# OpenDriveLab/ST-P3

Measured on AMD Instinct MI355X. Metric: BEV samples/sec (6-cam x 3-frame fwd+bwd), higher is better.
Workload: dtype bf16 convs / f32 voxel pool; 1 GPU; BASELINE configs[2]: batch=4/GPU, 6-cam 224x480, T=3, full STP3 fwd+bwd with segmentation + pedestrian + hdmap + depth CE + instance centerness/offset + flow losses, grad-clip 5, Adam; EfficientNet-B4, D=48, C=64, BEV 200x200; global_batch=4, parallelism=dp1, launch=hipgraph

## Files before the change

include/stp3_hip.h:

```cpp
#ifndef STP3_HIP_H
#define STP3_HIP_H

#include <stddef.h>
#include <stdint.h>

#ifdef __cplusplus
extern "C" {
#endif

#define STP3_OK          0
#define STP3_EINVAL   (-10001)
#define STP3_EUNSUP   (-10002)
#define STP3_ENOSPACE (-10003)

#define STP3_DTYPE_F32  0
#define STP3_DTYPE_BF16 1

typedef struct stp3_lift_dims {
    int32_t B, T, N;
    int32_t D, fH, fW;
    int32_t C;
    int32_t X, Y, Z;
} stp3_lift_dims;

// ... 99 lines not shown
    int32_t act, res_mode;
    int32_t has_sbias, has_oscale;
    int32_t cpad;
} stp3_bn_dims;

int stp3_bn_workspace_bytes(const stp3_bn_dims* dims, size_t* bytes);
int stp3_bn_stats(const stp3_bn_dims* dims, const void* x, const float* sbias, void* workspace,
                  size_t workspace_bytes, float* sums, void* stream);
int stp3_bn_apply_fwd(const stp3_bn_dims* dims, const void* x, const float* sbias, const void* res,
                      const float* oscale, const float* sums, double count, const float* gamma,
                      const float* beta, float eps, float momentum, float* running_mean,
                      float* running_var, float* save_mean, float* save_invstd, void* y, void* stream);
int stp3_bn_bwd_reduce(const stp3_bn_dims* dims, const void* dy, const void* x, const float* sbias,
                       const void* res, const float* oscale, const float* mean, const float* invstd,
                       const float* gamma, const float* beta, void* workspace, size_t workspace_bytes,
                       float* sample_sums, float* sums, void* stream);
int stp3_bn_apply_bwd(const stp3_bn_dims* dims, const void* dy, const void* x, const float* sbias,
                      const void* res, const float* oscale, const float* mean, const float* invstd,
                      const float* gamma, const float* beta, const float* sums, double count, void* dx,
                      void* dres, void* stream);
int stp3_bn_fwd_train(const stp3_bn_dims* dims, const void* x, const float* sbias, const void* res,
                      const float* oscale, const float* gamma, const float* beta, float eps, float momentum,
                      float* running_mean, float* running_var, float* stat_buf, void* workspace,
                      size_t workspace_bytes, void* y, void* stream);
int stp3_bn_bwd_train(const stp3_bn_dims* dims, const void* dy, const void* x, const float* sbias,
                      const void* res, const float* oscale, const float* mean, const float* invstd,
                      const float* gamma, const float* beta, void* workspace, size_t workspace_bytes,
                      float* sum_buf, void* dx, void* dres, void* stream);

int stp3_bn_dsbias(int32_t N, int32_t C, int32_t rows, const float* sample_sums, const float* gsums, double count,
                   const float* gamma, const float* invstd, float* dsbias, void* stream);
int stp3_sum_n(int32_t n, int64_t numel, int32_t dtype, const void* const* src, void* y, void* stream);
int stp3_sum_n_plane(int32_t n, int64_t numel, int32_t dtype, const void* const* src, const void* plane, int64_t per_sample,
                     int32_t C, void* y, void* stream);

int stp3_linear_fwd(int32_t M, int32_t K, int32_t N, const float* x, const float* w, int32_t ldw, const float* b, float* y,
                    void* stream);
int stp3_linear_bwd(int32_t M, int32_t K, int32_t N, const float* dy, const float* x, const float* w, int32_t ldw, float* dx,
                    float* dw, int32_t lddw, float* db, void* stream);

typedef struct stp3_conv_dims {
    int32_t N, H, W, Cin;
    int32_t Ho, Wo, Cout;
    int32_t KH, KW, stride;
    int32_t pad_h, pad_w, dil_h, dil_w;
    int32_t ldx, ldy;
    int32_t out_dtype, has_bias;
} stp3_conv_dims;

int stp3_conv2d_fwd_workspace(const stp3_conv_dims* dims, size_t* bytes);
int stp3_conv2d_fwd(const stp3_conv_dims* dims, const void* x, const void* w, const float* bias, void* y,
                    float* sums, void* workspace, size_t workspace_bytes, void* stream);

int stp3_conv2d_fwd_stats(const stp3_conv_dims* dims, const void* x, const void* w, float* sums, void* workspace,
                          size_t workspace_bytes, void* stream);
int stp3_conv2d_fwd_bnact(const stp3_conv_dims* dims, const void* x, const void* w, const float* coef, int32_t act, void* y,
                          void* stream);
int stp3_conv2d_bn_bwd_reduce(const stp3_conv_dims* dims, const void* x, const void* w, const void* dz, int32_t ldz,
                              const float* coef, int32_t act, float* sums, void* workspace, size_t workspace_bytes,
                              void* stream);
int stp3_conv2d_bn_bwd_apply(const stp3_conv_dims* dims, const void* x, const void* w, const void* dz, int32_t ldz,
                             const float* coef, int32_t act, const float* gsums, double count, void* dy, void* stream);
int stp3_conv2d_bn_bwd_apply_dx(const stp3_conv_dims* dims, const void* x, const void* w, const void* dz, int32_t ldz,
                                const float* coef, int32_t act, const float* gsums, double count, void* dy, void* dx,
                                int32_t lddx, const void* add, int32_t ldadd, void* stream);

int stp3_conv2d_fwd_add(const stp3_conv_dims* dims, const void* x, const void* w, const float* bias, const void* add,
                        int32_t ldadd, void* y, void* stream);

int stp3_conv2d_wgrad_workspace(const stp3_conv_dims* dims, size_t* bytes);
int stp3_conv2d_wgrad(const stp3_conv_dims* dims, const void* dy, const void* x, float* dw, void* workspace,
                      size_t workspace_bytes, void* stream);

#define STP3_WGRAD_BATCH_MAX 96
typedef struct stp3_wgrad_job {
    const void* partials;
    float* dw;
    int64_t numel;
    int32_t splits;
    int32_t reserved;
} stp3_wgrad_job;
int stp3_conv2d_wgrad_partials(const stp3_conv_dims* dims, const void* dy, const void* x, void* partials,
                               size_t partials_bytes, int32_t* splits, void* stream);
int stp3_conv2d_wgrad_reduce_batch(int32_t n, const stp3_wgrad_job* jobs, void* stream);

typedef struct stp3_se_dims {
    int32_t N, rows, C, ld;
    int32_t dtype;
} stp3_se_dims;

int stp3_se_workspace_bytes(const stp3_se_dims* dims, size_t* bytes);
int stp3_se_pool(const stp3_se_dims* dims, const void* x, const void* dy, void* workspace, size_t workspace_bytes,
                 float* out, void* stream);
int stp3_se_scale(const stp3_se_dims* dims, const void* x, const float* gate, const float* add, void* y, void* stream);

typedef struct stp3_se_mlp_dims {
    int32_t N, C, S;
    float inv_rows;
} stp3_se_mlp_dims;

int stp3_se_mlp_fwd(const stp3_se_mlp_dims* dims, const float* pooled_sum, const float* w1, const float* b1,
                    const float* w2, const float* b2, float* z1, float* gate, void* stream);
int stp3_se_mlp_bwd(const stp3_se_mlp_dims* dims, const float* dgate, const float* gate, const float* pooled_sum,
                    const float* z1, const float* w1, const float* w2, float* dz2, float* dz1, float* dpooled,
                    float* dw1, float* db1, float* dw2, float* db2, void* stream);

// ... 230 lines not shown
```

st-p3_amd/csrc/stp3_conv.hip:

```cpp
#include <hip/hip_runtime.h>
#include <stdint.h>
#include <stdlib.h>
#include <string.h>

#include "stp3_cdna.h"
#include "stp3_hip.h"

namespace {

typedef __attribute__((ext_vector_type(8))) __bf16 bf16x8;
typedef __attribute__((ext_vector_type(4))) float f32x4;
typedef __attribute__((ext_vector_type(16))) float f32x16;

struct ConvDims {
    int N, H, W, Cin, Ho, Wo, Cout;
    int KH, KW, stride, pad_h, pad_w, dil_h, dil_w;
    int ldx, ldy;
    int out_f32, has_bias;
    int M;
    int kchunks;
    int Ktot;
};

union Frag {
// ... 348 lines not shown
                *reinterpret_cast<uint4*>(yo + (size_t)m * d.ldy + co) =
                    make_uint4(pack_bf16(out[0], out[1]), pack_bf16(out[2], out[3]), pack_bf16(out[4], out[5]),
                               pack_bf16(out[6], out[7]));
            }
        }
    }
    if (MODE == kModeBwdReduce) {
        uint16_t* gt = tile + kBM * ldt;
        for (int e = tid; e < kBM * (BN / 8); e += 256) {
            const int p = e / (BN / 8), c = (e - p * (BN / 8)) * 8;
            const int m = m0 + p, co = co0 + c;
            uint4 g = make_uint4(0u, 0u, 0u, 0u);
            if (m < d.M && co < d.Cout) g = *reinterpret_cast<const uint4*>(ep.dz + (size_t)m * ep.ldz + co);
            *reinterpret_cast<uint4*>(gt + p * ldt + c) = g;
        }
        __syncthreads();
        float* red = reinterpret_cast<float*>(smem + 2 * kBM * ldt * 2);
        const int c = tid % BN, part = tid / BN;
        constexpr int kParts = 256 / BN, kRows = kBM / kParts;
        float s1 = 0.f, s2 = 0.f;
        if (co0 + c < d.Cout) {
            const float cs = ep.coef[co0 + c], ct = ep.coef[d.Cout + co0 + c];
            const float mu = ep.coef[2 * d.Cout + co0 + c], is = ep.coef[3 * d.Cout + co0 + c];
            for (int p = part * kRows; p < (part + 1) * kRows; ++p) {
                if (m0 + p < d.M) {
                    const float e0 = bf2f(tile[p * ldt + c]);
                    const float gg = bf2f(gt[p * ldt + c]) * epi_act_grad<ACT>(fmaf(e0, cs, ct));
                    s1 += gg;
                    s2 = fmaf(gg, (e0 - mu) * is, s2);
                }
            }
        }
        red[(part * 2) * BN + c] = s1;
        red[(part * 2 + 1) * BN + c] = s2;
        __syncthreads();
        if (tid < 2 * BN) {
            const int k = tid / BN, cc = tid - k * BN;
            float t = 0.f;
#pragma unroll
            for (int q = 0; q < kParts; ++q) t += red[(q * 2 + k) * BN + cc];
            if (co0 + cc < d.Cout) stat_partial[((size_t)tile_m * 2 + k) * d.Cout + co0 + cc] = t;
        }
    }
    if ((MODE == kModePlain || MODE == kModeStats) && stat_partial) {
        float* red = reinterpret_cast<float*>(smem + kBM * ldt * 2);
        const int c = tid % BN, part = tid / BN;
        constexpr int kParts = 256 / BN, kRows = kBM / kParts;
        float s1 = 0.f, s2 = 0.f;
        for (int p = part * kRows; p < (part + 1) * kRows; ++p) {
            if (m0 + p < d.M) {
                const float v = bf2f(tile[p * ldt + c]);
                s1 += v;
                s2 += v * v;
            }
        }
        red[(part * 2) * BN + c] = s1;
        red[(part * 2 + 1) * BN + c] = s2;
        __syncthreads();
        if (tid < 2 * BN) {
            const int k = tid / BN, cc = tid - k * BN;
            float t = 0.f;
#pragma unroll
            for (int q = 0; q < kParts; ++q) t += red[(q * 2 + k) * BN + cc];
            if (co0 + cc < d.Cout) stat_partial[((size_t)tile_m * 2 + k) * d.Cout + co0 + cc] = t;
        }
    }
}

struct Chan8 {
    stp3_f32x2 cs[4], ct[4], mu[4], is[4], a2[4], a3[4];
    uint32_t keep[4];
};

template <int MODE>
__device__ __forceinline__ void load_chan8(Chan8& k, const EpiArgs& ep, int Cout, int c, bool ok) {
#pragma unroll
    for (int r = 0; r < 4; ++r)
#pragma unroll
        for (int h = 0; h < 2; ++h) {
            k.cs[r][h] = k.ct[r][h] = k.mu[r][h] = k.is[r][h] = k.a2[r][h] = k.a3[r][h] = 0.f;
            if (MODE == kModeAffine && h == 0)
                k.keep[r] = (c + 2 * r < ep.cvalid ? 0x0000ffffu : 0u) | (c + 2 * r + 1 < ep.cvalid ? 0xffff0000u : 0u);
            if (MODE >= kModeBnAct && ok) {
                const int cc = c + 2 * r + h;
                k.cs[r][h] = ep.coef[cc];
                k.ct[r][h] = ep.coef[Cout + cc];
                if (MODE == kModeAffine) continue;
                k.mu[r][h] = ep.coef[2 * Cout + cc];
                k.is[r][h] = ep.coef[3 * Cout + cc];
                if (MODE == kModeBwdApply) {
                    const float k0 = ep.gsums[cc] * ep.inv_count, k1 = ep.gsums[Cout + cc] * ep.inv_count;
                    k.a2[r][h] = -(k.cs[r][h] * k.is[r][h]) * k1;
                    k.a3[r][h] = -k.cs[r][h] * k0 - k.a2[r][h] * k.mu[r][h];
                }
            }
        }
}

template <int MODE>
__device__ __forceinline__ void epi8(const uint32_t (&wds)[4], const uint32_t (&gds)[4], const Chan8& k, int act,
                                     stp3_f32x2 (&s1)[4], stp3_f32x2 (&s2)[4], uint32_t (&ow)[4], int res_mode = STP3_RES_NONE) {
#pragma unroll
    for (int r = 0; r < 4; ++r) {
        const uint32_t wd = MODE == kModeAffine ? wds[r] & k.keep[r] : wds[r];
        const stp3_f32x2 e0 = {__uint_as_float(wd << 16), __uint_as_float(wd & 0xffff0000u)};
        if (MODE == kModePlain || MODE == kModeStats) {
// ... 619 lines not shown
    }
    float4 t;
    t.x = (s0.x + s1.x) + (s2.x + s3.x); t.y = (s0.y + s1.y) + (s2.y + s3.y);
    t.z = (s0.z + s1.z) + (s2.z + s3.z); t.w = (s0.w + s1.w) + (s2.w + s3.w);
    red[threadIdx.x] = t;
    __syncthreads();
    if (kl == 0 && i < n) {
        const float4 a = red[cg], bb = red[64 + cg], c = red[128 + cg], d = red[192 + cg];
        float4 o;
        o.x = (a.x + bb.x) + (c.x + d.x); o.y = (a.y + bb.y) + (c.y + d.y);
        o.z = (a.z + bb.z) + (c.z + d.z); o.w = (a.w + bb.w) + (c.w + d.w);
        if (i + 3 < n && ((uintptr_t)(dw + i) & 15) == 0) {
            *reinterpret_cast<float4*>(dw + i) = o;
        } else {
            const float* oe = &o.x;
            for (int e = 0; e < 4 && i + e < n; ++e) dw[i + e] = oe[e];
        }
    }
}

inline int status() {
    hipError_t e = hipGetLastError();
    return e == hipSuccess ? STP3_OK : -(int)e;
}

inline size_t igemm_lds(int bn, int steps, bool out_f32) {
    const size_t stage = (size_t)(steps > 1 ? 2 : 1) * (kBM + bn) * kBK * 2;
    const size_t tile = out_f32 ? (size_t)kBM * (bn + 8) * 4 : (size_t)kBM * (bn + 8) * 2 + 512 * sizeof(float);
    return stage > tile ? stage : tile;
}

template <int TCO, int TCI>
int wgrad_launch(const ConvDims& d, int tco, int tci, int taps, int splits, int ksteps, int fold, const void* dy,
                 const void* x, void* workspace, hipStream_t s) {
    const size_t lds = (size_t)2 * (TCO + TCI) * kBK * 2;
    const int xcd = taps <= 9 && (int64_t)tco * tci * taps * splits < (1LL << 31);
    const bool buf = (size_t)d.M * d.ldy * 2 < (1ull << 31) && (size_t)d.N * d.H * d.W * d.ldx * 2 < (1ull << 31);
    if (buf) {
        hipError_t e = hipFuncSetAttribute(reinterpret_cast<const void*>(&conv2d_wgrad_kernel<TCO, TCI, true>),
                                           hipFuncAttributeMaxDynamicSharedMemorySize, (int)lds);
        if (e != hipSuccess) return -(int)e;
        hipLaunchKernelGGL((conv2d_wgrad_kernel<TCO, TCI, true>), dim3(tco * tci, taps, splits), dim3(256), lds, s, d, tci,
                           ksteps, fold, xcd, (const uint16_t*)dy, (const uint16_t*)x, (float*)workspace);
        return STP3_OK;
    }
    hipError_t e = hipFuncSetAttribute(reinterpret_cast<const void*>(&conv2d_wgrad_kernel<TCO, TCI>),
                                       hipFuncAttributeMaxDynamicSharedMemorySize, (int)lds);
    if (e != hipSuccess) return -(int)e;
    hipLaunchKernelGGL((conv2d_wgrad_kernel<TCO, TCI>), dim3(tco * tci, taps, splits), dim3(256), lds, s, d, tci, ksteps,
                       fold, xcd, (const uint16_t*)dy, (const uint16_t*)x, (float*)workspace);
    return STP3_OK;
}

}

extern "C" {

int stp3_conv2d_fwd_workspace(const stp3_conv_dims* p, size_t* bytes) {
    if (!p || !bytes || p->N <= 0 || p->Ho <= 0 || p->Wo <= 0 || p->Cout <= 0) return STP3_EINVAL;
    const int64_t M = (int64_t)p->N * p->Ho * p->Wo;
    const size_t parts = (size_t)((M + kBM - 1) / kBM);
    if (parts > 65536) return STP3_EUNSUP;
    *bytes = (parts + (parts + 255) / 256) * 2 * p->Cout * sizeof(float);
    return STP3_OK;
}

}

namespace {

template <int BN, int MODE, int ACT>
int igemm_launch_one(const ConvDims& d, dim3 grid, size_t lds, int tiles_co, const void* x, const void* w, const float* bias,
                     void* y, float* partial, const EpiArgs& ep, hipStream_t s) {
    const bool buf = (size_t)d.N * d.H * d.W * d.ldx * 2 < (1ull << 31) && (size_t)d.Cout * d.Ktot * 2 < (1ull << 31);
    if (buf) {
        hipError_t e = hipFuncSetAttribute(reinterpret_cast<const void*>(&conv2d_igemm_kernel<BN, MODE, ACT, true>),
                                           hipFuncAttributeMaxDynamicSharedMemorySize, (int)lds);
        if (e != hipSuccess) return -(int)e;
        hipLaunchKernelGGL((conv2d_igemm_kernel<BN, MODE, ACT, true>), grid, dim3(256), lds, s, d, tiles_co, (const uint16_t*)x,
                           (const uint16_t*)w, bias, y, partial, ep);
        return STP3_OK;
    }
    hipError_t e = hipFuncSetAttribute(reinterpret_cast<const void*>(&conv2d_igemm_kernel<BN, MODE, ACT>),
                                       hipFuncAttributeMaxDynamicSharedMemorySize, (int)lds);
    if (e != hipSuccess) return -(int)e;
    hipLaunchKernelGGL((conv2d_igemm_kernel<BN, MODE, ACT>), grid, dim3(256), lds, s, d, tiles_co, (const uint16_t*)x,
                       (const uint16_t*)w, bias, y, partial, ep);
    return STP3_OK;
}

template <int BN, int MODE>
int igemm_launch_act(int act, const ConvDims& d, dim3 grid, size_t lds, int tiles_co, const void* x, const void* w,
                     const float* bias, void* y, float* partial, const EpiArgs& ep, hipStream_t s) {
    if (MODE == kModePlain || MODE == kModeStats || act == STP3_ACT_NONE)
        return igemm_launch_one<BN, MODE, STP3_ACT_NONE>(d, grid, lds, tiles_co, x, w, bias, y, partial, ep, s);
    if (act == STP3_ACT_RELU) return igemm_launch_one<BN, MODE, STP3_ACT_RELU>(d, grid, lds, tiles_co, x, w, bias, y, partial, ep, s);
    return igemm_launch_one<BN, MODE, STP3_ACT_SWISH>(d, grid, lds, tiles_co, x, w, bias, y, partial, ep, s);
}

template <int PP, int KMAX, int MODE>
int pointwise_rows_launch_one(const ConvDims& d, int ksteps, int tiles_co, unsigned nwg, size_t lds, const void* x, const void* w,
                              void* y, float* partial, const EpiArgs& ep, hipStream_t s) {
    hipError_t e = hipFuncSetAttribute(reinterpret_cast<const void*>(&pointwise_rows_kernel<PP, KMAX, MODE>),
                                       hipFuncAttributeMaxDynamicSharedMemorySize, (int)lds);
    if (e != hipSuccess) return -(int)e;
    hipLaunchKernelGGL((pointwise_rows_kernel<PP, KMAX, MODE>), dim3(nwg), dim3(256), lds, s, d, ksteps, tiles_co,
                       (const uint16_t*)x, (const uint16_t*)w, (uint16_t*)y, partial, ep);
    return STP3_OK;
}

template <int PP, int KMAX>
int pointwise_rows_launch_mode(int mode, const ConvDims& d, int ksteps, int tiles_co, unsigned nwg, size_t lds, const void* x,
                               const void* w, void* y, float* partial, const EpiArgs& ep, hipStream_t s) {
    switch (mode) {
        case kModePlain: return pointwise_rows_launch_one<PP, KMAX, kModePlain>(d, ksteps, tiles_co, nwg, lds, x, w, y, partial, ep, s);
        case kModeStats: return pointwise_rows_launch_one<PP, KMAX, kModeStats>(d, ksteps, tiles_co, nwg, lds, x, w, y, partial, ep, s);
        case kModeBnAct: return pointwise_rows_launch_one<PP, KMAX, kModeBnAct>(d, ksteps, tiles_co, nwg, lds, x, w, y, partial, ep, s);
        case kModeAffine: return pointwise_rows_launch_one<PP, KMAX, kModeAffine>(d, ksteps, tiles_co, nwg, lds, x, w, y, partial, ep, s);
        case kModeBwdReduce:
            return pointwise_rows_launch_one<PP, KMAX, kModeBwdReduce>(d, ksteps, tiles_co, nwg, lds, x, w, y, partial, ep, s);
        default: return pointwise_rows_launch_one<PP, KMAX, kModeBwdApply>(d, ksteps, tiles_co, nwg, lds, x, w, y, partial, ep, s);
    }
}

template <int KMAX, int MODE>
int pointwise_direct_launch_one(const ConvDims& d, int ksteps, unsigned gx, int* parts, const void* x, const void* w, void* y,
                                float* partial, const EpiArgs& ep, hipStream_t s) {
    static const int resident = [] {
        int per_cu = 0;
        if (hipOccupancyMaxActiveBlocksPerMultiprocessor(&per_cu, pointwise_direct_kernel<KMAX, MODE>, 256, 0) != hipSuccess || per_cu < 1)
            per_cu = 1;
        return per_cu * 256;
    }();
    const int cblocks = (d.Cout + 31) / 32;
    const int ntiles = (d.M + 31) / 32;
    int ngroups = resident * 4 / cblocks;
    if (ngroups > (int)gx) ngroups = (int)gx;
    if (ngroups > ntiles) ngroups = ntiles;
    if (ngroups < 1) ngroups = 1;
    *parts = ngroups;
// ... 9 lines not shown
    switch (mode) {
        case kModePlain: return pointwise_direct_launch_one<KMAX, kModePlain>(d, ksteps, gx, parts, x, w, y, partial, ep, s);
        case kModeStats: return pointwise_direct_launch_one<KMAX, kModeStats>(d, ksteps, gx, parts, x, w, y, partial, ep, s);
        case kModeBnAct: return pointwise_direct_launch_one<KMAX, kModeBnAct>(d, ksteps, gx, parts, x, w, y, partial, ep, s);
        case kModeAffine: return pointwise_direct_launch_one<KMAX, kModeAffine>(d, ksteps, gx, parts, x, w, y, partial, ep, s);
        case kModeBwdReduce: return pointwise_direct_launch_one<KMAX, kModeBwdReduce>(d, ksteps, gx, parts, x, w, y, partial, ep, s);
        default: return pointwise_direct_launch_one<KMAX, kModeBwdApply>(d, ksteps, gx, parts, x, w, y, partial, ep, s);
    }
}

constexpr int kPointwiseMaxCin = 128;

bool pointwise_applies(const stp3_conv_dims* p, const void* y) {
    return p->KH == 1 && p->KW == 1 && p->stride == 1 && p->pad_h == 0 && p->pad_w == 0 && p->H == p->Ho && p->W == p->Wo &&
           p->Cin <= kPointwiseMaxCin && p->Cout >= 64 && !p->has_bias && p->out_dtype == STP3_DTYPE_BF16 &&
           p->Cout % 8 == 0 && p->ldy % 8 == 0 && !((uintptr_t)y & 15);
}

int pointwise_run(const ConvDims& d, const void* x, const void* w, void* y, float* sums, float* partial, unsigned gx,
                  hipStream_t s, int mode, const EpiArgs& ep) {
    const int ksteps = (d.Cin + 15) / 16;
    int rc, parts;
    const bool rows_small = (d.Cout == 144 || d.Cout == 192) && ksteps <= 2;
    const bool rows_lines = d.Cout % 64 == 0;
    if ((rows_small || rows_lines) && d.ldy % 8 == 0 && (!mode_bwd(mode) || ep.ldz % 8 == 0)) {
        const int pp = rows_small ? d.Cout / 8 : (d.Cout % 128 == 0 ? 16 : 8), nt = (pp + 3) / 4;
        const int tiles_co = d.Cout / (pp * 8);
        if (ep.dx && !(rows_small && mode == kModeBwdApply && d.Cin <= 32)) return STP3_EUNSUP;
        const size_t lds = (size_t)nt * 32 * (ksteps * 16 + 8) * 2 + (size_t)4 * 32 * (nt * 32 + 8) * 2 +
                           (ep.dx ? (size_t)32 * (nt * 32 + 8) * 2 : 0);
        unsigned per_cu = (unsigned)((160 * 1024) / lds);
        if (per_cu > 3) per_cu = 3;
        unsigned groups = (256 * per_cu + tiles_co - 1) / tiles_co;
        if (groups > gx) groups = gx;
        parts = (int)groups;
        const unsigned nwg = groups * (unsigned)tiles_co;
        if (pp == 18) rc = pointwise_rows_launch_mode<18, 2>(mode, d, ksteps, tiles_co, nwg, lds, x, w, y, partial, ep, s);
        else if (pp == 24) rc = pointwise_rows_launch_mode<24, 2>(mode, d, ksteps, tiles_co, nwg, lds, x, w, y, partial, ep, s);
        else if (pp == 8) rc = pointwise_rows_launch_mode<8, 8>(mode, d, ksteps, tiles_co, nwg, lds, x, w, y, partial, ep, s);
        else if (ksteps <= 4) rc = pointwise_rows_launch_mode<16, 4>(mode, d, ksteps, tiles_co, nwg, lds, x, w, y, partial, ep, s);
        else rc = pointwise_rows_launch_mode<16, 8>(mode, d, ksteps, tiles_co, nwg, lds, x, w, y, partial, ep, s);
    } else {
        if (ep.dx) return STP3_EUNSUP;
        if (ksteps <= 2) rc = pointwise_direct_launch_mode<2>(mode, d, ksteps, gx, &parts, x, w, y, partial, ep, s);
        else if (ksteps <= 4) rc = pointwise_direct_launch_mode<4>(mode, d, ksteps, gx, &parts, x, w, y, partial, ep, s);
        else rc = pointwise_direct_launch_mode<8>(mode, d, ksteps, gx, &parts, x, w, y, partial, ep, s);
    }
    if (rc) return rc;
    if (sums) launch_colsum(s, parts, 2 * d.Cout, partial, sums);
    return status();
}

int igemm_run(const stp3_conv_dims* p, const void* x, const void* w, const float* bias, void* y, float* sums, void* workspace,
              size_t workspace_bytes, void* stream, int mode, int act, EpiArgs ep) {
    if (!p || !x || !w || (mode != kModeStats && mode != kModeBwdReduce && !y)) return STP3_EINVAL;
    if (p->N <= 0 || p->H <= 0 || p->W <= 0 || p->Cin <= 0 || p->Cout <= 0 || p->Ho <= 0 || p->Wo <= 0 || p->KH <= 0 ||
        p->KW <= 0 || p->stride <= 0 || p->dil_h <= 0 || p->dil_w <= 0 || p->pad_h < 0 || p->pad_w < 0)
        return STP3_EINVAL;
    if (p->has_bias && !bias) return STP3_EINVAL;
    if (p->Cin % 8 || p->ldx % 8 || p->ldx < p->Cin || p->ldy < p->Cout) return STP3_EUNSUP;
    if (((uintptr_t)x & 15) || ((uintptr_t)w & 15)) return STP3_EUNSUP;
    if (p->out_dtype != STP3_DTYPE_BF16 && p->out_dtype != STP3_DTYPE_F32) return STP3_EUNSUP;
    if (y && ((uintptr_t)y & (p->out_dtype == STP3_DTYPE_F32 ? 3 : 1))) return STP3_EUNSUP;
    if ((sums || mode != kModePlain) && p->out_dtype != STP3_DTYPE_BF16) return STP3_EUNSUP;
    if (mode != kModePlain) {
        if ((p->has_bias && mode != kModeAffine) || p->Cout % 8 || p->ldy % 8 || (y && ((uintptr_t)y & 15))) return STP3_EUNSUP;
        if (mode >= kModeBnAct && !ep.coef) return STP3_EINVAL;
        if (mode == kModeAffine && ep.res && (ep.ldres % 8 || ep.ldres < p->Cout || ((uintptr_t)ep.res & 15))) return STP3_EUNSUP;
        if (mode_bwd(mode) && (!ep.dz || ep.ldz % 8 || ep.ldz < p->Cout || ((uintptr_t)ep.dz & 15))) return STP3_EUNSUP;
        if (mode == kModeBwdApply && !ep.gsums) return STP3_EINVAL;
        if ((mode == kModeStats || mode == kModeBwdReduce) && !sums) return STP3_EINVAL;
    }
    const int64_t M = (int64_t)p->N * p->Ho * p->Wo;
    if (M >= (1LL << 31) || (int64_t)p->N * p->H * p->W >= (1LL << 31)) return STP3_EUNSUP;
    ConvDims d;
    d.N = p->N; d.H = p->H; d.W = p->W; d.Cin = p->Cin; d.Ho = p->Ho; d.Wo = p->Wo; d.Cout = p->Cout;
    d.KH = p->KH; d.KW = p->KW; d.stride = p->stride; d.pad_h = p->pad_h; d.pad_w = p->pad_w;
    d.dil_h = p->dil_h; d.dil_w = p->dil_w; d.ldx = p->ldx; d.ldy = p->ldy;
    d.out_f32 = p->out_dtype == STP3_DTYPE_F32; d.has_bias = p->has_bias;
    d.M = (int)M; d.kchunks = (p->Cin + 31) / 32; d.Ktot = p->KH * p->KW * p->Cin;
    const unsigned gx = (unsigned)((M + kBM - 1) / kBM);
    hipStream_t s = (hipStream_t)stream;
    float* partial = nullptr;
    if (sums) {
        if (gx > 65536) return STP3_EUNSUP;
        if (!workspace || workspace_bytes < ((size_t)gx + (gx + 255) / 256) * 2 * p->Cout * sizeof(float)) return STP3_ENOSPACE;
        partial = (float*)workspace;
    }
    if (y && ((uintptr_t)y & 15)) return STP3_EUNSUP;
    if (ep.dx) {
        if (!pointwise_applies(p, y) || ep.lddx % 4 || ep.lddx < p->Cin || ((uintptr_t)ep.dx & 7) ||
            (ep.add && (ep.ldadd % 4 || ep.ldadd < p->Cin || ((uintptr_t)ep.add & 7))))
            return STP3_EUNSUP;
        ep.act = act;
        return pointwise_run(d, x, w, y, sums, partial, gx, s, mode, ep);
    }
    if (ep.add) {
        if (mode != kModePlain || d.out_f32 || p->Cout % 8 || p->ldy % 8 || ep.ldadd % 8 || ep.ldadd < p->Cout ||
            ((uintptr_t)ep.add & 15) || ((uintptr_t)y & 15))
            return STP3_EUNSUP;
    } else if (pointwise_applies(p, y)) {
        if (ep.sbias) return STP3_EUNSUP;
        ep.act = act;
        return pointwise_run(d, x, w, y, sums, partial, gx, s, mode, ep);
    }
    const int steps = (d.Ktot + kBK - 1) / kBK;
    const bool wide = p->Cout > 64 && steps > 2 && (int64_t)gx * ((p->Cout + 127) / 128) >= 512;
    const int bn = wide ? 128 : 64;
    size_t lds = igemm_lds(bn, steps, d.out_f32 != 0);
    if (mode == kModeBwdReduce) {
        const size_t need = (size_t)2 * kBM * (bn + 8) * 2 + 512 * sizeof(float);
        if (need > lds) lds = need;
    }
    const int tiles_co = (p->Cout + bn - 1) / bn;
    if ((int64_t)gx * tiles_co >= (1LL << 31)) return STP3_EUNSUP;
    const dim3 grid(gx * (unsigned)tiles_co);
    int rc;
#define STP3_IGEMM_MODE(MODE)                                                                                                \
    rc = wide ? igemm_launch_act<128, MODE>(act, d, grid, lds, tiles_co, x, w, bias, y, partial, ep, s)                       \
              : igemm_launch_act<64, MODE>(act, d, grid, lds, tiles_co, x, w, bias, y, partial, ep, s)
    switch (mode) {
        case kModePlain: STP3_IGEMM_MODE(kModePlain); break;
        case kModeStats: STP3_IGEMM_MODE(kModeStats); break;
        case kModeBnAct: STP3_IGEMM_MODE(kModeBnAct); break;
        case kModeAffine: STP3_IGEMM_MODE(kModeAffine); break;
        case kModeBwdReduce: STP3_IGEMM_MODE(kModeBwdReduce); break;
        default: STP3_IGEMM_MODE(kModeBwdApply); break;
    }
#undef STP3_IGEMM_MODE
    if (rc) return rc;
    if (sums) launch_colsum(s, (int)gx, 2 * p->Cout, partial, sums);
    return status();
}

}

extern "C" {

int stp3_conv2d_fwd(const stp3_conv_dims* p, const void* x, const void* w, const float* bias, void* y, float* sums,
                    void* workspace, size_t workspace_bytes, void* stream) {
    return igemm_run(p, x, w, bias, y, sums, workspace, workspace_bytes, stream, kModePlain, STP3_ACT_NONE, EpiArgs());
}

int stp3_conv2d_fwd_add(const stp3_conv_dims* p, const void* x, const void* w, const float* bias, const void* add, int32_t ldadd,
                        void* y, void* stream) {
    if (!add) return STP3_EINVAL;
    EpiArgs ep = EpiArgs();
    ep.add = (const uint16_t*)add;
    ep.ldadd = ldadd;
    return igemm_run(p, x, w, bias, y, nullptr, nullptr, 0, stream, kModePlain, STP3_ACT_NONE, ep);
}

int stp3_conv2d_fwd_stats(const stp3_conv_dims* p, const void* x, const void* w, float* sums, void* workspace,
                          size_t workspace_bytes, void* stream) {
    return igemm_run(p, x, w, nullptr, nullptr, sums, workspace, workspace_bytes, stream, kModeStats, STP3_ACT_NONE, EpiArgs());
}

int stp3_conv2d_fwd_bnact(const stp3_conv_dims* p, const void* x, const void* w, const float* coef, int32_t act, void* y,
                          void* stream) {
    EpiArgs ep = EpiArgs();
    ep.coef = coef;
    return igemm_run(p, x, w, nullptr, y, nullptr, nullptr, 0, stream, kModeBnAct, act, ep);
}

int stp3_conv2d_fwd_affine(const stp3_conv_dims* p, const void* x, const void* w, const float* bias, const float* coef,
                           const float* sbias, int32_t channels, int32_t act, const void* res, int32_t ldres, int32_t res_mode,
                           void* y, void* stream) {
    if (!p || !coef) return STP3_EINVAL;
    if (act != STP3_ACT_NONE && act != STP3_ACT_RELU && act != STP3_ACT_SWISH) return STP3_EINVAL;
    if (res_mode != STP3_RES_NONE && res_mode != STP3_RES_BEFORE_ACT && res_mode != STP3_RES_AFTER_ACT) return STP3_EINVAL;
    if ((res_mode != STP3_RES_NONE) != (res != nullptr)) return STP3_EINVAL;
    if (channels <= 0 || channels > p->Cout) return STP3_EINVAL;
    if (p->Cout != (channels + 7) / 8 * 8) return STP3_EUNSUP;
    EpiArgs ep = EpiArgs();
    ep.coef = coef; ep.res = (const uint16_t*)res; ep.ldres = ldres; ep.res_mode = res_mode; ep.cvalid = channels;
    ep.sbias = sbias; ep.hw = p->Ho > 0 && p->Wo > 0 ? p->Ho * p->Wo : 1;
    return igemm_run(p, x, w, bias, y, nullptr, nullptr, 0, stream, kModeAffine, act, ep);
}

int stp3_conv2d_bn_bwd_reduce(const stp3_conv_dims* p, const void* x, const void* w, const void* dz, int32_t ldz,
                              const float* coef, int32_t act, float* sums, void* workspace, size_t workspace_bytes,
                              void* stream) {
    EpiArgs ep = EpiArgs();
    ep.coef = coef; ep.dz = (const uint16_t*)dz; ep.ldz = ldz;
    return igemm_run(p, x, w, nullptr, nullptr, sums, workspace, workspace_bytes, stream, kModeBwdReduce, act, ep);
}

int stp3_conv2d_bn_bwd_apply(const stp3_conv_dims* p, const void* x, const void* w, const void* dz, int32_t ldz,
                             const float* coef, int32_t act, const float* gsums, double count, void* dy, void* stream) {
    if (!(count >= 1.0)) return STP3_EINVAL;
    EpiArgs ep = EpiArgs();
    ep.coef = coef; ep.dz = (const uint16_t*)dz; ep.ldz = ldz; ep.gsums = gsums; ep.inv_count = (float)(1.0 / count);
    return igemm_run(p, x, w, nullptr, dy, nullptr, nullptr, 0, stream, kModeBwdApply, act, ep);
}
// ... 133 lines not shown
```

st-p3_amd/stp3_amd/_lib.py:

```python
import ctypes
import os

from . import profiling

_HERE = os.path.dirname(os.path.abspath(__file__))
LIB_PATH = os.path.join(_HERE, 'libstp3hip.so')

c_void_p = ctypes.c_void_p
c_int = ctypes.c_int
c_int32 = ctypes.c_int32
c_float = ctypes.c_float
c_size_t = ctypes.c_size_t


class LiftDims(ctypes.Structure):
    _fields_ = [(k, ctypes.c_int32) for k in ('B', 'T', 'N', 'D', 'fH', 'fW', 'C', 'X', 'Y', 'Z')]

    @property
    def BT(self):
        return self.B * self.T

    @property
    def NPIX(self):
        return self.N * self.fH * self.fW
# ... 134 lines not shown
ACT_NONE, ACT_RELU, ACT_SWISH = 0, 1, 2
ACT_GELU = 3
RES_NONE, RES_BEFORE_ACT, RES_AFTER_ACT = 0, 1, 2

_DIMS_P = ctypes.POINTER(LiftDims)
_BN_P = ctypes.POINTER(BnDims)
c_double = ctypes.c_double
_DW_P = ctypes.POINTER(DwConvDims)
_LN_P = ctypes.POINTER(LayerNormDims)
_GRU_P = ctypes.POINTER(GruDims)

SIGNATURES = {
    'stp3_version': (ctypes.c_char_p, []),
    'stp3_voxel_index': (c_int, [_DIMS_P] + [c_void_p] * 9 + [c_int, c_void_p, c_void_p, c_void_p]),
    'stp3_lift_plan_bytes': (c_int, [_DIMS_P, ctypes.POINTER(c_size_t)]),
    'stp3_lift_plan_build': (c_int, [_DIMS_P] + [c_void_p] * 12 + [c_size_t, c_void_p]),
    'stp3_depth_softmax': (c_int, [_DIMS_P, c_void_p, c_void_p, c_void_p]),
    'stp3_lift_workspace_bytes': (c_int, [_DIMS_P, ctypes.POINTER(c_size_t)]),
    'stp3_lift_splat_fwd': (c_int, [_DIMS_P, c_void_p, c_void_p, c_void_p, c_float, c_int, c_void_p, c_size_t,
                                    c_void_p, c_void_p, c_void_p]),
    'stp3_lift_bwd_needs_prob': (c_int, [_DIMS_P, ctypes.POINTER(c_int)]),
    'stp3_lift_splat_bwd': (c_int, [_DIMS_P, c_void_p, c_int, c_int, c_void_p, c_void_p, c_void_p, c_void_p, c_void_p,
                                    c_float, c_void_p, c_size_t, c_void_p, c_void_p, c_void_p]),
    'stp3_gru_reset_cat_fwd': (c_int, [_GRU_P, c_void_p, c_void_p, c_void_p, c_void_p]),
    'stp3_gru_output_fwd': (c_int, [_GRU_P, c_void_p, c_void_p, c_void_p, c_void_p, c_void_p]),
    'stp3_gru_output_bwd': (c_int, [_GRU_P, c_void_p, ctypes.c_int32, c_void_p, c_void_p, c_void_p, c_void_p, c_void_p, c_void_p]),
    'stp3_gru_reset_cat_bwd': (c_int, [_GRU_P, c_void_p, ctypes.c_int32, c_void_p, c_void_p, c_void_p, c_void_p, c_void_p, c_void_p]),
    'stp3_layernorm_fwd': (c_int, [_LN_P, c_void_p, c_void_p, c_void_p, c_void_p, c_void_p]),
    'stp3_layernorm_bwd_workspace': (c_int, [_LN_P, ctypes.POINTER(c_size_t)]),
    'stp3_layernorm_bwd': (c_int, [_LN_P] + [c_void_p] * 8 + [c_size_t, c_void_p]),
    'stp3_dwconv2d_fwd': (c_int, [_DW_P, c_void_p, c_void_p, c_void_p, c_void_p]),
    'stp3_dwconv2d_fwd_bias': (c_int, [_DW_P, c_void_p, c_void_p, c_void_p, c_void_p, c_void_p]),
    'stp3_dwconv2d_bwd_data': (c_int, [_DW_P, c_void_p, c_void_p, c_void_p, c_void_p]),
    'stp3_dwconv2d_bwd_weight_workspace': (c_int, [_DW_P, ctypes.POINTER(c_size_t)]),
    'stp3_dwconv2d_bwd_weight': (c_int, [_DW_P, c_void_p, c_void_p, c_void_p, c_void_p, c_size_t, c_void_p]),
    'stp3_dwconv2d_bwd_weight_oihw': (c_int, [_DW_P, c_void_p, c_void_p, c_void_p, c_void_p, c_size_t, c_void_p]),
    'stp3_bn_workspace_bytes': (c_int, [_BN_P, ctypes.POINTER(c_size_t)]),
    'stp3_bn_stats': (c_int, [_BN_P, c_void_p, c_void_p, c_void_p, c_size_t, c_void_p, c_void_p]),
    'stp3_bn_apply_fwd': (c_int, [_BN_P] + [c_void_p] * 5 + [c_double, c_void_p, c_void_p, c_float, c_float]
                          + [c_void_p] * 6),
    'stp3_bn_bwd_reduce': (c_int, [_BN_P] + [c_void_p] * 10 + [c_size_t, c_void_p, c_void_p, c_void_p]),
    'stp3_bn_apply_bwd': (c_int, [_BN_P] + [c_void_p] * 10 + [c_double, c_void_p, c_void_p, c_void_p]),
    'stp3_bn_fwd_train': (c_int, [_BN_P] + [c_void_p] * 6 + [c_float, c_float] + [c_void_p] * 4 + [c_size_t, c_void_p,
                                                                                                 c_void_p]),
    'stp3_bn_bwd_train': (c_int, [_BN_P] + [c_void_p] * 10 + [c_size_t] + [c_void_p] * 4),
    'stp3_bn_dsbias': (c_int, [c_int32, c_int32, c_int32, c_void_p, c_void_p, c_double, c_void_p, c_void_p, c_void_p, c_void_p]),
    'stp3_sum_n': (c_int, [c_int32, ctypes.c_int64, c_int32, c_void_p, c_void_p, c_void_p]),
    'stp3_linear_fwd': (c_int, [c_int32, c_int32, c_int32, c_void_p, c_void_p, c_int32, c_void_p, c_void_p, c_void_p]),
    'stp3_linear_bwd': (c_int, [c_int32, c_int32, c_int32, c_void_p, c_void_p, c_void_p, c_int32, c_void_p, c_void_p, c_int32, c_void_p,
                                c_void_p]),
    'stp3_sum_n_plane': (c_int, [c_int32, ctypes.c_int64, c_int32, c_void_p, c_void_p, ctypes.c_int64, c_int32, c_void_p, c_void_p]),
    'stp3_conv2d_fwd_workspace': (c_int, [ctypes.POINTER(ConvDims), ctypes.POINTER(c_size_t)]),
    'stp3_conv2d_fwd': (c_int, [ctypes.POINTER(ConvDims)] + [c_void_p] * 6 + [c_size_t, c_void_p]),
    'stp3_conv2d_fwd_add': (c_int, [ctypes.POINTER(ConvDims), c_void_p, c_void_p, c_void_p, c_void_p, c_int32, c_void_p, c_void_p]),
    'stp3_conv2d_fwd_stats': (c_int, [ctypes.POINTER(ConvDims), c_void_p, c_void_p, c_void_p, c_void_p, c_size_t, c_void_p]),
    'stp3_conv2d_fwd_bnact': (c_int, [ctypes.POINTER(ConvDims), c_void_p, c_void_p, c_void_p, c_int32, c_void_p, c_void_p]),
    'stp3_conv2d_bn_bwd_reduce': (c_int, [ctypes.POINTER(ConvDims), c_void_p, c_void_p, c_void_p, c_int32, c_void_p, c_int32,
                                          c_void_p, c_void_p, c_size_t, c_void_p]),
    'stp3_conv2d_bn_bwd_apply': (c_int, [ctypes.POINTER(ConvDims), c_void_p, c_void_p, c_void_p, c_int32, c_void_p, c_int32,
                                         c_void_p, c_double, c_void_p, c_void_p]),
    'stp3_se_workspace_bytes': (c_int, [ctypes.POINTER(SeDims), ctypes.POINTER(c_size_t)]),
    'stp3_se_pool': (c_int, [ctypes.POINTER(SeDims), c_void_p, c_void_p, c_void_p, c_size_t, c_void_p, c_void_p]),
    'stp3_se_scale': (c_int, [ctypes.POINTER(SeDims), c_void_p, c_void_p, c_void_p, c_void_p, c_void_p]),
    'stp3_conv2d_bn_bwd_apply_dx': (c_int, [ctypes.POINTER(ConvDims), c_void_p, c_void_p, c_void_p, c_int32, c_void_p, c_int32, c_void_p,
                                            ctypes.c_double, c_void_p, c_void_p, c_int32, c_void_p, c_int32, c_void_p]),
    'stp3_conv2d_wgrad_workspace': (c_int, [ctypes.POINTER(ConvDims), ctypes.POINTER(c_size_t)]),
    'stp3_conv2d_wgrad': (c_int, [ctypes.POINTER(ConvDims), c_void_p, c_void_p, c_void_p, c_void_p, c_size_t, c_void_p]),
    'stp3_conv2d_wgrad_partials': (c_int, [ctypes.POINTER(ConvDims), c_void_p, c_void_p, c_void_p, c_size_t,
                                           ctypes.POINTER(c_int32), c_void_p]),
    'stp3_conv2d_wgrad_reduce_batch': (c_int, [c_int32, ctypes.POINTER(WgradJob), c_void_p]),
    'stp3_conv2d_prep_weights': (c_int, [c_void_p, c_int32, ctypes.c_int64, c_void_p]),
    'stp3_conv2d_scatter_weight_grads': (c_int, [c_void_p, c_int32, ctypes.c_int64, c_void_p]),
    'stp3_se_mlp_fwd': (c_int, [c_void_p] * 9),
    'stp3_se_mlp_bwd': (c_int, [c_void_p] * 15),
    'stp3_optim_workspace_bytes': (c_int, [ctypes.c_int64, ctypes.POINTER(c_size_t)]),
    'stp3_optim_clip_adam': (c_int, [c_void_p, c_int32, ctypes.c_int64] + [c_float] * 6 + [c_void_p, c_void_p, c_size_t,
                                                                                          c_void_p]),
    'stp3_causal_pair_fwd': (c_int, [ctypes.POINTER(PairDims), c_void_p, c_void_p, c_void_p]),
    'stp3_causal_pair_bwd': (c_int, [ctypes.POINTER(PairDims), c_void_p, c_void_p, c_void_p]),
    'stp3_upsample_bilinear_fwd': (c_int, [ctypes.POINTER(UpsampleDims), c_void_p, c_void_p, c_void_p]),
    'stp3_upsample_bilinear_bwd': (c_int, [ctypes.POINTER(UpsampleDims), c_void_p, c_void_p, c_void_p]),
    'stp3_dwconv2d_fwd_stats_workspace': (c_int, [_DW_P, ctypes.POINTER(c_size_t)]),
    'stp3_dwconv2d_fwd_stats': (c_int, [_DW_P, c_void_p, c_void_p, c_void_p, c_void_p, c_void_p, c_size_t, c_void_p]),
    'stp3_bn_finalize': (c_int, [c_void_p, c_int32, c_double, c_void_p, c_void_p, c_float, c_float, c_void_p, c_void_p,
                                 c_void_p, c_void_p]),
    'stp3_mbconv_workspace_bytes': (c_int, [ctypes.POINTER(SeDims), ctypes.POINTER(c_size_t)]),
    'stp3_se_pool_act': (c_int, [ctypes.POINTER(SeDims), c_void_p, c_void_p, c_void_p, c_int32, c_void_p, c_size_t, c_void_p,
                                 c_void_p]),
    'stp3_mbconv_scale_act': (c_int, [ctypes.POINTER(SeDims), c_int32, c_void_p, c_void_p, c_void_p, c_int32, c_void_p,
                                      c_void_p, c_void_p]),
    'stp3_mbconv_bwd_reduce': (c_int, [ctypes.POINTER(SeDims), c_int32, c_void_p, c_void_p, c_void_p, c_int32, c_void_p,
                                       c_size_t, c_void_p, c_void_p]),
    'stp3_mbconv_bwd_coef': (c_int, [c_int32, c_int32, c_void_p, c_void_p, c_void_p, c_void_p, c_void_p]),
    'stp3_mbconv_bwd_apply': (c_int, [ctypes.POINTER(SeDims), c_int32, c_void_p, c_void_p, c_void_p, c_int32, c_void_p,
                                      c_void_p, c_void_p, c_double, c_void_p, c_void_p]),
    'stp3_dwconv2d_fwd_stats_bn': (c_int, [_DW_P, c_void_p, c_void_p, c_void_p, c_void_p, c_double, c_void_p, c_void_p, c_float,
                                           c_float, c_void_p, c_void_p, c_void_p, c_void_p, c_size_t, c_void_p]),
    'stp3_ce_topk_workspace_bytes': (c_int, [ctypes.POINTER(CeDims), ctypes.POINTER(c_size_t)]),
    'stp3_ce_topk_fwd': (c_int, [ctypes.POINTER(CeDims)] + [c_void_p] * 6 + [c_double, c_int32, c_void_p, c_void_p, c_size_t,
                                                                           c_void_p]),
    'stp3_ce_topk_bwd': (c_int, [ctypes.POINTER(CeDims)] + [c_void_p] * 7 + [c_double, c_void_p, c_void_p]),
    'stp3_reg_loss_workspace_bytes': (c_int, [ctypes.POINTER(c_size_t)]),
    'stp3_reg_loss_fwd': (c_int, [c_int32] * 4 + [c_float, c_int32] + [c_void_p] * 5 + [c_size_t, c_void_p]),
    'stp3_reg_loss_bwd': (c_int, [c_int32] * 4 + [c_float, c_int32] + [c_void_p] * 7),
    'stp3_warp_nearest': (c_int, [c_int32] * 4 + [c_void_p] * 5),
    'stp3_traj_cost_fwd': (c_int, [ctypes.POINTER(PlanDims)] + [c_void_p] * 14),
# ... 73 lines not shown
```

Measured before the change: 112.7 samples/s.

## Add halo-tiled 3x3 conv forward kernel staging input patch in LDS for small maps

Adds a specialized 3x3 stride-1 conv forward kernel that loads an 8x16 output tile plus a one-pixel halo of input once into LDS and walks the nine taps by offsetting into that patch. Weights are double-buffered from global memory. It is meant to remove the repeated im2col-style input gathers of the generic implicit-GEMM path. It is routed only for plain and stats modes with Cin<=128 and small maps (N*H*W<4096). Larger LDS use may reduce occupancy, and a tiled fallback entry point is exposed.

```diff
diff --git a/include/stp3_hip.h b/include/stp3_hip.h
--- a/include/stp3_hip.h
+++ b/include/stp3_hip.h
@@ -175,6 +175,12 @@
 int stp3_conv2d_fwd(const stp3_conv_dims* dims, const void* x, const void* w, const float* bias, void* y,
                     float* sums, void* workspace, size_t workspace_bytes, void* stream);
 
+#define STP3_CONV_ROUTE_TILED 0
+#define STP3_CONV_ROUTE_HALO  1
+int stp3_conv2d_fwd_route(const stp3_conv_dims* dims);
+int stp3_conv2d_fwd_tiled(const stp3_conv_dims* dims, const void* x, const void* w, const float* bias, void* y,
+                          float* sums, void* workspace, size_t workspace_bytes, void* stream);
+
 int stp3_conv2d_fwd_stats(const stp3_conv_dims* dims, const void* x, const void* w, float* sums, void* workspace,
                           size_t workspace_bytes, void* stream);
 int stp3_conv2d_fwd_bnact(const stp3_conv_dims* dims, const void* x, const void* w, const float* coef, int32_t act, void* y,
diff --git a/st-p3_amd/csrc/stp3_conv.hip b/st-p3_amd/csrc/stp3_conv.hip
--- a/st-p3_amd/csrc/stp3_conv.hip
+++ b/st-p3_amd/csrc/stp3_conv.hip
@@ -424,6 +424,204 @@
                 const float v = bf2f(tile[p * ldt + c]);
                 s1 += v;
                 s2 += v * v;
+            }
+        }
+        red[(part * 2) * BN + c] = s1;
+        red[(part * 2 + 1) * BN + c] = s2;
+        __syncthreads();
+        if (tid < 2 * BN) {
+            const int k = tid / BN, cc = tid - k * BN;
+            float t = 0.f;
+#pragma unroll
+            for (int q = 0; q < kParts; ++q) t += red[(q * 2 + k) * BN + cc];
+            if (co0 + cc < d.Cout) stat_partial[((size_t)tile_m * 2 + k) * d.Cout + co0 + cc] = t;
+        }
+    }
+}
+
+constexpr int kHaloTH = 8, kHaloTW = 16;
+constexpr int kHaloW = kHaloTW + 2;
+constexpr int kHaloPix = (kHaloTH + 2) * kHaloW;
+constexpr int kHaloMaxCin = 128;
+constexpr int kHaloSmallMaps = 4096;
+
+template <int BN, int MODE>
+__global__ __launch_bounds__(256) void conv2d_halo3x3_kernel(ConvDims d, int tiles_co, int tiles_h, int tiles_w,
+                                                             const uint16_t* __restrict__ x, const uint16_t* __restrict__ w,
+                                                             const float* __restrict__ bias, uint16_t* __restrict__ yo,
+                                                             float* __restrict__ stat_partial, EpiArgs ep) {
+    static_assert(kHaloTH * kHaloTW == kBM, "tile");
+    constexpr int TP = BN == 128 ? 2 : 1;
+    constexpr int TC = 2;
+    constexpr int kWStage = BN * kBK * 2;
+    extern __shared__ __attribute__((aligned(16))) uint8_t smem[];
+    const int tid = threadIdx.x;
+    const int lane = tid & 63;
+    const int wave = __builtin_amdgcn_readfirstlane(tid >> 6);
+    const int wm = BN == 128 ? (wave >> 1) : wave;
+    const int wn = BN == 128 ? (wave & 1) : 0;
+    const int v = xcd_order(blockIdx.x, gridDim.x);
+    const int tile_m = v / tiles_co, tile_co = v - tile_m * tiles_co;
+    const int tw = tile_m % tiles_w, tq = tile_m / tiles_w;
+    const int th = tq % tiles_h, n = tq / tiles_h;
+    const int h0 = th * kHaloTH, w0 = tw * kHaloTW;
+    const int co0 = tile_co * BN;
+    const int pitch = d.Cin * 2 + 16;
+    uint8_t* const wimg = smem + kHaloPix * pitch;
+
+    {
+        const stp3_buffer xbuf = make_buffer(x, (uint32_t)((size_t)d.N * d.H * d.W * d.ldx * 2));
+        const int pc = tid & 15;
+        const bool pc_ok = pc < (d.Cin >> 3);
+#pragma unroll
+        for (int p0 = 0; p0 < kHaloPix; p0 += 64) {
+            u32x4 r[4];
+#pragma unroll
+            for (int i = 0; i < 4; ++i) {
+                const int pix = p0 + 16 * i + (tid >> 4);
+                const int hr = pix / kHaloW, hc = pix - hr * kHaloW;
+                const int hi = h0 - 1 + hr, wi = w0 - 1 + hc;
+                const bool ok = pc_ok & (pix < kHaloPix) & ((unsigned)hi < (unsigned)d.H) & ((unsigned)wi < (unsigned)d.W);
+                r[i] = buffer_load16(xbuf, ok ? (uint32_t)(((n * d.H + hi) * d.W + wi) * d.ldx + pc * 8) * 2u : kBufOob);
+            }
+#pragma unroll
+            for (int i = 0; i < 4; ++i) {
+                const int pix = p0 + 16 * i + (tid >> 4);
+                if (pc_ok && pix < kHaloPix) *reinterpret_cast<u32x4*>(smem + pix * pitch + pc * 16) = r[i];
+            }
+        }
+    }
+
+    const int j = tid & 7, rr = tid >> 3;
+    const stp3_buffer wbuf = make_buffer(w, (uint32_t)((size_t)d.Cout * d.Ktot * 2));
+    uint32_t woff[BN / 32];
+#pragma unroll
+    for (int i = 0; i < BN / 32; ++i) {
+        const int co = co0 + rr + 32 * i;
+        woff[i] = co < d.Cout ? (uint32_t)(co * d.Ktot) * 2u : kBufOob;
+    }
+    int kk = j * 8;
+    u32x4 rb[BN / 32];
+    auto load_w = [&]() {
+        const bool kvalid = kk < d.Ktot;
+#pragma unroll
+        for (int i = 0; i < BN / 32; ++i)
+            rb[i] = buffer_load16(wbuf, (kvalid & (woff[i] != kBufOob)) ? woff[i] + (uint32_t)kk * 2u : kBufOob);
+        kk += kBK;
+    };
+    auto store_w = [&](uint8_t* buf) {
+#pragma unroll
+        for (int i = 0; i < BN / 32; ++i) *reinterpret_cast<u32x4*>(buf + lds_piece(rr + 32 * i, j)) = rb[i];
+    };
+
+    f32x16 acc[TC][TP];
+#pragma unroll
+    for (int a = 0; a < TC; ++a)
+#pragma unroll
+        for (int b = 0; b < TP; ++b)
+#pragma unroll
+            for (int r = 0; r < 16; ++r) acc[a][b][r] = 0.f;
+
+    const int frow = lane & 31, fk = lane >> 5;
+    const int fquad = frow >> 2;
+    const int fpix = ((0x96 >> fquad) & 1) * 16 + (fquad >> 1) * 4 + (frow & 3);
+    int pbase[TP];
+#pragma unroll
+    for (int b = 0; b < TP; ++b) {
+        const int p = wm * (32 * TP) + b * 32 + fpix;
+        pbase[b] = ((p >> 4) * kHaloW + (p & 15)) * pitch + fk * 16;
+    }
+    const int chunks = d.Ktot >> 4;
+    const int steps = (chunks + 3) >> 2;
+    load_w();
+    store_w(wimg);
+    __syncthreads();
+    int toff = 0, ci = 0, kw = 0;
+    for (int s = 0; s < steps; ++s) {
+        const uint8_t* cur = wimg + (s & 1) * kWStage;
+        if (s + 1 < steps) load_w();
+#pragma unroll
+        for (int ks = 0; ks < kBK / 16; ++ks) {
+            const int t = s * (kBK / 16) + ks < chunks ? toff : 0;
+            Frag fa[TC], fb[TP];
+#pragma unroll
+            for (int a = 0; a < TC; ++a)
+                fa[a].u = *reinterpret_cast<const uint4*>(cur + lds_piece(wn * 64 + a * 32 + frow, ks * 2 + fk));
+#pragma unroll
+            for (int b = 0; b < TP; ++b) fb[b].u = *reinterpret_cast<const uint4*>(smem + pbase[b] + t);
+#pragma unroll
+            for (int a = 0; a < TC; ++a)
+#pragma unroll
+                for (int b = 0; b < TP; ++b)
+                    acc[a][b] = __builtin_amdgcn_mfma_f32_32x32x16_bf16(fa[a].v, fb[b].v, acc[a][b], 0, 0, 0);
+            ci += 16;
+            const bool tap_done = ci == d.Cin;
+            const bool row_done = tap_done & (kw == 2);
+            ci = tap_done ? 0 : ci;
+            kw = row_done ? 0 : kw + (tap_done ? 1 : 0);
+            toff += 32 + (tap_done ? 16 : 0) + (row_done ? (kHaloW - 3) * pitch : 0);
+        }
+        if (s + 1 < steps) store_w(wimg + ((s + 1) & 1) * kWStage);
+        __syncthreads();
+    }
+
+    const int ldt = BN + 8;
+    uint16_t* tile = reinterpret_cast<uint16_t*>(smem);
+#pragma unroll
+    for (int a = 0; a < TC; ++a)
+#pragma unroll
+        for (int b = 0; b < TP; ++b)
+#pragma unroll
+            for (int q = 0; q < 4; ++q) {
+                const int c = wn * 64 + a * 32 + 8 * q + 4 * fk;
+                const int p = wm * (32 * TP) + b * 32 + fpix;
+                float vv[4] = {acc[a][b][4 * q], acc[a][b][4 * q + 1], acc[a][b][4 * q + 2], acc[a][b][4 * q + 3]};
+                if (d.has_bias) {
+#pragma unroll
+                    for (int r = 0; r < 4; ++r) vv[r] += co0 + c + r < d.Cout ? bias[co0 + c + r] : 0.f;
+                }
+                *reinterpret_cast<uint2*>(tile + p * ldt + c) = make_uint2(pack_bf16(vv[0], vv[1]), pack_bf16(vv[2], vv[3]));
+            }
+    __syncthreads();
+    auto in_image = [&](int p) { return h0 + (p >> 4) < d.H && w0 + (p & 15) < d.W; };
+    if (MODE == kModePlain) {
+        for (int e = tid; e < kBM * (BN / 8); e += 256) {
+            const int p = e / (BN / 8), c = (e - p * (BN / 8)) * 8;
+            const int co = co0 + c;
+            if (!in_image(p) || co >= d.Cout) continue;
+            const int m = (n * d.H + h0 + (p >> 4)) * d.W + w0 + (p & 15);
+            uint4 o = *reinterpret_cast<const uint4*>(tile + p * ldt + c);
+            uint16_t* dst = yo + (size_t)m * d.ldy + co;
+            if (co + 7 < d.Cout && (d.ldy & 7) == 0) {
+                if (ep.add) {
+                    const uint4 g = *reinterpret_cast<const uint4*>(ep.add + (size_t)m * ep.ldadd + co);
+                    const uint32_t vw[4] = {o.x, o.y, o.z, o.w}, aw[4] = {g.x, g.y, g.z, g.w};
+                    uint32_t ow[4];
+#pragma unroll
+                    for (int r = 0; r < 4; ++r)
+                        ow[r] = pack_bf16(__uint_as_float(vw[r] << 16) + __uint_as_float(aw[r] << 16),
+                                          __uint_as_float(vw[r] & 0xffff0000u) + __uint_as_float(aw[r] & 0xffff0000u));
+                    o = make_uint4(ow[0], ow[1], ow[2], ow[3]);
+                }
+                *reinterpret_cast<uint4*>(dst) = o;
+            } else {
+                const uint32_t wds[4] = {o.x, o.y, o.z, o.w};
+#pragma unroll
+                for (int r = 0; r < 8; ++r)
+                    if (co + r < d.Cout) dst[r] = (uint16_t)(wds[r >> 1] >> (16 * (r & 1)));
+            }
+        }
+    }
+    if (stat_partial) {
+        float* red = reinterpret_cast<float*>(smem + kBM * ldt * 2);
+        const int c = tid % BN, part = tid / BN;
+        constexpr int kParts = 256 / BN, kRows = kBM / kParts;
+        float s1 = 0.f, s2 = 0.f;
+        for (int p = part * kRows; p < (part + 1) * kRows; ++p) {
+            if (in_image(p)) {
+                const float t = bf2f(tile[p * ldt + c]);
+                s1 += t;
+                s2 += t * t;
             }
         }
         red[(part * 2) * BN + c] = s1;
@@ -1149,14 +1347,32 @@
     return STP3_OK;
 }
 
+bool halo_geometry(const stp3_conv_dims* p) {
+    return p->KH == 3 && p->KW == 3 && p->stride == 1 && p->dil_h == 1 && p->dil_w == 1 && p->pad_h == 1 && p->pad_w == 1 &&
+           p->Ho == p->H && p->Wo == p->W && p->Cin % 16 == 0 && p->Cin <= kHaloMaxCin && p->out_dtype == STP3_DTYPE_BF16 &&
+           (int64_t)p->N * p->H * p->W * p->ldx * 2 < (1LL << 31) && (int64_t)p->Cout * 9 * p->Cin * 2 < (1LL << 31);
+}
+int64_t halo_tiles(const stp3_conv_dims* p) {
+    return (int64_t)p->N * ((p->H + kHaloTH - 1) / kHaloTH) * ((p->W + kHaloTW - 1) / kHaloTW);
+}
+bool halo_listed(const stp3_conv_dims* p) {
+    return (int64_t)p->N * p->H * p->W < kHaloSmallMaps;
+}
+
 }
 
 extern "C" {
+
+int stp3_conv2d_fwd_route(const stp3_conv_dims* p) {
+    if (!p) return STP3_EINVAL;
+    return halo_geometry(p) && halo_listed(p) ? STP3_CONV_ROUTE_HALO : STP3_CONV_ROUTE_TILED;
+}
 
 int stp3_conv2d_fwd_workspace(const stp3_conv_dims* p, size_t* bytes) {
     if (!p || !bytes || p->N <= 0 || p->Ho <= 0 || p->Wo <= 0 || p->Cout <= 0) return STP3_EINVAL;
     const int64_t M = (int64_t)p->N * p->Ho * p->Wo;
-    const size_t parts = (size_t)((M + kBM - 1) / kBM);
+    size_t parts = (size_t)((M + kBM - 1) / kBM);
+    if (halo_geometry(p) && (size_t)halo_tiles(p) > parts) parts = (size_t)halo_tiles(p);
     if (parts > 65536) return STP3_EUNSUP;
     *bytes = (parts + (parts + 255) / 256) * 2 * p->Cout * sizeof(float);
     return STP3_OK;
@@ -1183,6 +1399,21 @@
     if (e != hipSuccess) return -(int)e;
     hipLaunchKernelGGL((conv2d_igemm_kernel<BN, MODE, ACT>), grid, dim3(256), lds, s, d, tiles_co, (const uint16_t*)x,
                        (const uint16_t*)w, bias, y, partial, ep);
+    return STP3_OK;
+}
+
+template <int BN, int MODE>
+int halo_launch(const ConvDims& d, unsigned tiles, int tiles_co, const void* x, const void* w, const float* bias, void* y,
+                float* partial, const EpiArgs& ep, hipStream_t s) {
+    size_t lds = (size_t)kHaloPix * (d.Cin * 2 + 16) + 2 * (size_t)BN * kBK * 2;
+    const size_t epi = (size_t)kBM * (BN + 8) * 2 + 512 * sizeof(float);
+    if (epi > lds) lds = epi;
+    hipError_t e = hipFuncSetAttribute(reinterpret_cast<const void*>(&conv2d_halo3x3_kernel<BN, MODE>),
+                                       hipFuncAttributeMaxDynamicSharedMemorySize, (int)lds);
+    if (e != hipSuccess) return -(int)e;
+    const int tiles_h = (d.H + kHaloTH - 1) / kHaloTH, tiles_w = (d.W + kHaloTW - 1) / kHaloTW;
+    hipLaunchKernelGGL((conv2d_halo3x3_kernel<BN, MODE>), dim3(tiles * (unsigned)tiles_co), dim3(256), lds, s, d, tiles_co, tiles_h,
+                       tiles_w, (const uint16_t*)x, (const uint16_t*)w, bias, (uint16_t*)y, partial, ep);
     return STP3_OK;
 }
 
@@ -1298,7 +1529,7 @@
 }
 
 int igemm_run(const stp3_conv_dims* p, const void* x, const void* w, const float* bias, void* y, float* sums, void* workspace,
-              size_t workspace_bytes, void* stream, int mode, int act, EpiArgs ep) {
+              size_t workspace_bytes, void* stream, int mode, int act, EpiArgs ep, bool per_tap = false) {
     if (!p || !x || !w || (mode != kModeStats && mode != kModeBwdReduce && !y)) return STP3_EINVAL;
     if (p->N <= 0 || p->H <= 0 || p->W <= 0 || p->Cin <= 0 || p->Cout <= 0 || p->Ho <= 0 || p->Wo <= 0 || p->KH <= 0 ||
         p->KW <= 0 || p->stride <= 0 || p->dil_h <= 0 || p->dil_w <= 0 || p->pad_h < 0 || p->pad_w < 0)
@@ -1327,10 +1558,14 @@
     d.M = (int)M; d.kchunks = (p->Cin + 31) / 32; d.Ktot = p->KH * p->KW * p->Cin;
     const unsigned gx = (unsigned)((M + kBM - 1) / kBM);
     hipStream_t s = (hipStream_t)stream;
+    const bool halo = !per_tap && (mode == kModePlain || mode == kModeStats) && halo_geometry(p) && halo_listed(p) &&
+                      halo_tiles(p) * ((p->Cout + 63) / 64) < (1LL << 31);
+    const unsigned parts = halo ? (unsigned)halo_tiles(p) : gx;
     float* partial = nullptr;
     if (sums) {
-        if (gx > 65536) return STP3_EUNSUP;
-        if (!workspace || workspace_bytes < ((size_t)gx + (gx + 255) / 256) * 2 * p->Cout * sizeof(float)) return STP3_ENOSPACE;
+        if (parts > 65536) return STP3_EUNSUP;
+        if (!workspace || workspace_bytes < ((size_t)parts + (parts + 255) / 256) * 2 * p->Cout * sizeof(float))
+            return STP3_ENOSPACE;
         partial = (float*)workspace;
     }
     if (y && ((uintptr_t)y & 15)) return STP3_EUNSUP;
@@ -1349,6 +1584,20 @@
         if (ep.sbias) return STP3_EUNSUP;
         ep.act = act;
         return pointwise_run(d, x, w, y, sums, partial, gx, s, mode, ep);
+    }
+    if (halo) {
+        const bool wide_h = p->Cout > 64 && (int64_t)parts * ((p->Cout + 127) / 128) >= 512;
+        const int tiles_co = (p->Cout + (wide_h ? 127 : 63)) / (wide_h ? 128 : 64);
+        int rc;
+        if (mode == kModeStats)
+            rc = wide_h ? halo_launch<128, kModeStats>(d, parts, tiles_co, x, w, bias, y, partial, ep, s)
+                        : halo_launch<64, kModeStats>(d, parts, tiles_co, x, w, bias, y, partial, ep, s);
+        else
+            rc = wide_h ? halo_launch<128, kModePlain>(d, parts, tiles_co, x, w, bias, y, partial, ep, s)
+                        : halo_launch<64, kModePlain>(d, parts, tiles_co, x, w, bias, y, partial, ep, s);
+        if (rc) return rc;
+        if (sums) launch_colsum(s, (int)parts, 2 * p->Cout, partial, sums);
+        return status();
     }
     const int steps = (d.Ktot + kBK - 1) / kBK;
     const bool wide = p->Cout > 64 && steps > 2 && (int64_t)gx * ((p->Cout + 127) / 128) >= 512;
@@ -1386,6 +1635,11 @@
 int stp3_conv2d_fwd(const stp3_conv_dims* p, const void* x, const void* w, const float* bias, void* y, float* sums,
                     void* workspace, size_t workspace_bytes, void* stream) {
     return igemm_run(p, x, w, bias, y, sums, workspace, workspace_bytes, stream, kModePlain, STP3_ACT_NONE, EpiArgs());
+}
+
+int stp3_conv2d_fwd_tiled(const stp3_conv_dims* p, const void* x, const void* w, const float* bias, void* y, float* sums,
+                          void* workspace, size_t workspace_bytes, void* stream) {
+    return igemm_run(p, x, w, bias, y, sums, workspace, workspace_bytes, stream, kModePlain, STP3_ACT_NONE, EpiArgs(), true);
 }
 
 int stp3_conv2d_fwd_add(const stp3_conv_dims* p, const void* x, const void* w, const float* bias, const void* add, int32_t ldadd,
diff --git a/st-p3_amd/stp3_amd/_lib.py b/st-p3_amd/stp3_amd/_lib.py
--- a/st-p3_amd/stp3_amd/_lib.py
+++ b/st-p3_amd/stp3_amd/_lib.py
@@ -210,6 +210,8 @@
     'stp3_sum_n_plane': (c_int, [c_int32, ctypes.c_int64, c_int32, c_void_p, c_void_p, ctypes.c_int64, c_int32, c_void_p, c_void_p]),
     'stp3_conv2d_fwd_workspace': (c_int, [ctypes.POINTER(ConvDims), ctypes.POINTER(c_size_t)]),
     'stp3_conv2d_fwd': (c_int, [ctypes.POINTER(ConvDims)] + [c_void_p] * 6 + [c_size_t, c_void_p]),
+    'stp3_conv2d_fwd_tiled': (c_int, [ctypes.POINTER(ConvDims)] + [c_void_p] * 6 + [c_size_t, c_void_p]),
+    'stp3_conv2d_fwd_route': (c_int, [ctypes.POINTER(ConvDims)]),
     'stp3_conv2d_fwd_add': (c_int, [ctypes.POINTER(ConvDims), c_void_p, c_void_p, c_void_p, c_void_p, c_int32, c_void_p, c_void_p]),
     'stp3_conv2d_fwd_stats': (c_int, [ctypes.POINTER(ConvDims), c_void_p, c_void_p, c_void_p, c_void_p, c_size_t, c_void_p]),
     'stp3_conv2d_fwd_bnact': (c_int, [ctypes.POINTER(ConvDims), c_void_p, c_void_p, c_void_p, c_int32, c_void_p, c_void_p]),
```

Result: no change. 112.6 samples/s (-0.1%).
